# WHDY/SceneDepthEstimation

Hardware: AMD Instinct MI355X
Metric: Mpixel-disparities/sec (H*W*D cost voxels per second, end-to-end per pair) (higher is better)
Workload: dtype f32; 1 GPU; north_star; H=1024, W=1024, D=192, C=64, nlayers=5, pipeline=tower+cv_wta, global_batch=1, parallelism=pairdp1

## Files before the change

scenedepthestimation_amd/csrc/cv_row.hip:

```cpp
#include "cv_cert.h"

#include <algorithm>
#include <type_traits>

namespace sde {

constexpr int RW_S = 8;
constexpr float RW_SCALE = 256.0f;
constexpr float RW_K = 1.5e-5f;
constexpr float RW_ABS = 9.3132257e-10f;
constexpr float RW_NMAX = 127.0f;
typedef _Float16 rw_f16x8 __attribute__((ext_vector_type(8)));

__device__ __forceinline__ void rw_split(float x, _Float16 &h, _Float16 &l)
{
    const float xs = x * RW_SCALE;
    h = (_Float16)xs;
    l = (_Float16)(xs - (float)h);
}

constexpr int RW_T = 32;
constexpr int RW_WAVES = 8;
constexpr int RW_NX = RW_T * RW_WAVES;
constexpr int RW_NEW = RW_NX / RW_T;
// ... 244 lines not shown
#if CV_FASTSPLIT & 32
        const float xs[4] = {v[i].x * RW_SCALE, v[i].y * RW_SCALE, v[i].z * RW_SCALE, v[i].w * RW_SCALE};
        typedef _Float16 h2 __attribute__((ext_vector_type(2)));
        uint32_t hw[2], lw[2];
#pragma unroll
        for (int e = 0; e < 2; e++) {
            const h2 hh = {(_Float16)xs[2 * e], (_Float16)xs[2 * e + 1]};
            hw[e] = __builtin_bit_cast(uint32_t, hh);
            asm("v_fma_mixlo_f16 %0, %1, 1.0, -%2 op_sel_hi:[0,0,1]" : "=&v"(lw[e]) : "v"(xs[2 * e]), "v"(hw[e]));
            asm("v_fma_mixhi_f16 %0, %1, 1.0, -%2 op_sel:[0,0,1] op_sel_hi:[0,0,1]" : "+v"(lw[e]) : "v"(xs[2 * e + 1]), "v"(hw[e]));
        }
        *reinterpret_cast<uint2 *>(base) = uint2{hw[0], hw[1]};
        *reinterpret_cast<uint2 *>(base + 256 * 16) = uint2{lw[0], lw[1]};
#else
        _Float16 h0, h1, h2, h3, l0, l1, l2, l3;
        rw_split(v[i].x, h0, l0); rw_split(v[i].y, h1, l1); rw_split(v[i].z, h2, l2); rw_split(v[i].w, h3, l3);
        typedef _Float16 h4 __attribute__((ext_vector_type(4)));
        const h4 hv = {h0, h1, h2, h3}, lv = {l0, l1, l2, l3};
        *reinterpret_cast<uint2 *>(base) = __builtin_bit_cast(uint2, hv);
        *reinterpret_cast<uint2 *>(base + 256 * 16) = __builtin_bit_cast(uint2, lv);
#endif
        float ss = v[i].x * v[i].x + v[i].y * v[i].y + v[i].z * v[i].z + v[i].w * v[i].w;
        ss += rw_dpp<0xB1>(ss);
        ss += rw_dpp<0x4E>(ss);
        ss += rw_dpp<0x141>(ss);
        ss += rw_dpp<0x140>(ss);
        mx = max(mx, __float_as_uint(ss));
#if CV_FASTSPLIT & 16
        bad |= rw_nonfinite(ss);
#else
        bad |= rw_nonfinite(v[i].x) || rw_nonfinite(v[i].y) || rw_nonfinite(v[i].z) || rw_nonfinite(v[i].w);
#endif
    }
#pragma unroll
    for (int o = 1; o < 64; o <<= 1) mx = max(mx, (unsigned)__shfl_xor((int)mx, o, 64));
    const bool anybad = __ballot(bad) != 0;
    if (lane == 0) {
        tmax[slot] = mx;
        tbad[slot] = anybad ? 1u : 0u;
    }
}

template <bool WANT_MIN>
__global__ __launch_bounds__(512) void cv_wta_row2_kernel(const float *__restrict__ fl, const float *__restrict__ fr,
                                                          int H, int W, int d0, int d1, int tlo0, int nw, int nt,
                                                          float *__restrict__ out_min, int32_t *__restrict__ out_arg,
                                                          float *__restrict__ out_disp, unsigned *__restrict__ counter,
                                                          int32_t *__restrict__ list, const float *__restrict__ prev_min)
{
    extern __shared__ __attribute__((aligned(16))) uint4 rsm2[];
    uint4 *ring = rsm2;
    unsigned *tmax = reinterpret_cast<unsigned *>(ring + nt * 512);
    unsigned *tbad = tmax + nt;
    const int y = blockIdx.x;
    const int tid = threadIdx.x, lane = tid & 63;
    const int wave = __builtin_amdgcn_readfirstlane(tid >> 6);
    const int j = lane & 31, h = lane >> 5;
    const float *flrow = fl + (size_t)y * W * 64;
    const float *frrow = fr + (size_t)y * W * 64;
    const size_t rowpix = (size_t)y * W;
    const int nss = (W + R2_NX - 1) / R2_NX;
    auto slot_of = [&](int T) { int r = T % nt; return r < 0 ? r + nt : r; };

    if (wave >= 4) {
        const int sw = wave - 4;
        constexpr int PB = 4;
        float4 nv[8];
#pragma unroll
        for (int b = 0; b < 4 / PB; b++) {
            float4 pv[PB][8];
#pragma unroll
            for (int i = 0; i < PB; i++)
                if (sw + 4 * (PB * b + i) < nw) r2_load(frrow, W, tlo0 + sw + 4 * (PB * b + i), lane, pv[i]);
            if (b == 4 / PB - 1 && nss > 1) r2_load(frrow, W, tlo0 + nw + sw, lane, nv);
#pragma unroll
            for (int i = 0; i < PB; i++)
                if (sw + 4 * (PB * b + i) < nw) r2_store(ring, tmax, tbad, slot_of(tlo0 + sw + 4 * (PB * b + i)), lane, pv[i]);
        }
        __syncthreads();
        for (int k = 0; k < nss; k++) {
            if (k + 1 < nss) {
                const int T = tlo0 + R2_NEW * (k + 1) + nw - R2_NEW + sw;
                r2_store(ring, tmax, tbad, slot_of(T), lane, nv);
                if (k + 2 < nss) r2_load(frrow, W, T + R2_NEW, lane, nv);
            }
            __syncthreads();
        }
        return;
    }

    const int grp = wave & 3;
    float4 lraw[8];
    auto load_left = [&](int kk) {
        const int xx = kk * R2_NX + RW_T * grp + j;
        const float4 *src = reinterpret_cast<const float4 *>(flrow) + (size_t)(xx < W ? xx : 0) * 16 + 2 * h;
#pragma unroll
        for (int s2 = 0; s2 < 4; s2++) { lraw[2 * s2] = src[4 * s2]; lraw[2 * s2 + 1] = src[4 * s2 + 1]; }
    };
    load_left(0);
    __syncthreads();

    for (int k = 0; k < nss; k++) {
        const int tlo = tlo0 + R2_NEW * k;
        const bool more = k + 1 < nss;
        const int xb = k * R2_NX + RW_T * grp;
        const int x = xb + j;
        const bool xok = x < W;
        float best = -__builtin_inff(), second = -__builtin_inff();
        float wcost = -0.0f;
        int arg = -1;
        float nl = 0.0f;
        unsigned nmax2 = 0u, wbad = 0u;
        bool lbad = false;
        if (xb < W && xb + RW_T - 1 < d0) {
            if (more) load_left(k + 1);
        } else if (xb < W) {
            rw_f16x8 bh[4], bl[4];
            float ssl = 0.0f;
#if CV_FASTSPLIT & 1
            const float scl = RW_SCALE;
#pragma unroll
            for (int s2 = 0; s2 < 4; s2++) {
                const float4 a = lraw[2 * s2], b = lraw[2 * s2 + 1];
                const float v8[8] = {a.x, a.y, a.z, a.w, b.x, b.y, b.z, b.w};
                uint32_t hw[4], lw[4];
#pragma unroll
                for (int e = 0; e < 8; e += 2) {
                    const float x0 = v8[e] * scl, x1 = v8[e + 1] * scl;
                    typedef _Float16 h2 __attribute__((ext_vector_type(2)));
                    const h2 hh = {(_Float16)x0, (_Float16)x1};
                    const uint32_t hv = __builtin_bit_cast(uint32_t, hh);
                    uint32_t lv;
                    asm("v_fma_mixlo_f16 %0, %1, 1.0, -%2 op_sel_hi:[0,0,1]" : "=&v"(lv) : "v"(x0), "v"(hv));
                    asm("v_fma_mixhi_f16 %0, %1, 1.0, -%2 op_sel:[0,0,1] op_sel_hi:[0,0,1]" : "+v"(lv) : "v"(x1), "v"(hv));
                    hw[e / 2] = hv;
                    lw[e / 2] = lv;
                    ssl += v8[e] * v8[e];
                    ssl += v8[e + 1] * v8[e + 1];
                }
                bh[s2] = __builtin_bit_cast(rw_f16x8, uint4{hw[0], hw[1], hw[2], hw[3]});
                bl[s2] = __builtin_bit_cast(rw_f16x8, uint4{lw[0], lw[1], lw[2], lw[3]});
            }
#else
#pragma unroll
            for (int s2 = 0; s2 < 4; s2++) {
                const float4 a = lraw[2 * s2], b = lraw[2 * s2 + 1];
                const float v8[8] = {a.x, a.y, a.z, a.w, b.x, b.y, b.z, b.w};
#pragma unroll
                for (int e = 0; e < 8; e++) {
                    _Float16 hh, ll;
                    rw_split(v8[e], hh, ll);
                    bh[s2][e] = hh;
                    bl[s2][e] = ll;
                    ssl += v8[e] * v8[e];
                    if (!(CV_FASTSPLIT & 2)) lbad |= rw_nonfinite(v8[e]);
                }
            }
#endif
#if CV_FASTSPLIT & 2
#if CV_FASTSPLIT & 8
            ssl += __shfl_xor(ssl, 32, 64);
#else
            ssl += __builtin_bit_cast(float, __builtin_amdgcn_permlane32_swap(__float_as_uint(ssl), __float_as_uint(ssl),
                                                                              false, false)[1]);
#endif
            lbad = rw_nonfinite(ssl);
#else
            ssl += __shfl_xor(ssl, 32, 64);
            lbad |= __shfl_xor((int)lbad, 32, 64) != 0;
#endif
            nl = sqrtf(ssl) * FX_NORM_UP;
            if (more) load_left(k + 1);

            float b1[4], b2[4];
            int ag[4];
#pragma unroll
            for (int t = 0; t < 4; t++) { b1[t] = -__builtin_inff(); b2[t] = -__builtin_inff(); ag[t] = -1; }
            const int Ta = (xb - d1 + 1 + RW_T * 4096) / RW_T - 4096;
            const int Tb = (xb + 31 - d0 + RW_T * 4096) / RW_T - 4096;
            const int T0 = max(Ta, tlo), T1 = min(Tb, tlo + nw - 1);
            int slot = slot_of(T0);
            {
                const int n = T1 - T0 + 1;
                constexpr int PD = 1;
                rw_f16x8 fh[PD][4], fo[PD][4];
                fx_floatx16 A[2];
                auto nxt = [&](int sl2) { return sl2 + 1 == nt ? 0 : sl2 + 1; };
                auto frag = [&](int sl2, rw_f16x8 (&ah)[4], rw_f16x8 (&al)[4]) {
                    const uint4 *tp = ring + sl2 * 512;
#pragma unroll
                    for (int s2 = 0; s2 < 4; s2++) {
                        const int sl = fx_slot(j, 2 * s2 + h);
                        ah[s2] = __builtin_bit_cast(rw_f16x8, tp[sl]);
                        al[s2] = __builtin_bit_cast(rw_f16x8, tp[256 + sl]);
                    }
                };
                auto mfma = [&](int m, fx_floatx16 &acc, const rw_f16x8 (&ah)[4], const rw_f16x8 (&al)[4]) {
                    if (m == 0) acc = __builtin_amdgcn_mfma_f32_32x32x16_f16(al[0], bh[0], fx_floatx16{0}, 0, 0, 0);
                    else if (m < 8) acc = __builtin_amdgcn_mfma_f32_32x32x16_f16((m & 1) ? ah[m >> 1] : al[m >> 1],
                                                                                (m & 1) ? bl[m >> 1] : bh[m >> 1],
                                                                                acc, 0, 0, 0);
                    else acc = __builtin_amdgcn_mfma_f32_32x32x16_f16(ah[m - 8], bh[m - 8], acc, 0, 0, 0);
                };
                auto score1 = [&](const fx_floatx16 &acc, int r, auto mode_c, const int (&dk)[4]) {
                    constexpr int MODE = decltype(mode_c)::value;
                    const int tt = r & 3;
                    const bool in = MODE == 0   ? true
                                    : MODE == 1 ? dk[r >> 2] < d1 + tt
                                    : MODE == 3 ? dk[r >> 2] >= d0 + tt
                                                : (dk[r >> 2] - tt) >= d0 && (dk[r >> 2] - tt) < d1;
                    const float sc = in ? acc[r] : -__builtin_inff();
                    const bool gt = sc > b1[tt];
                    ag[tt] = gt ? dk[r >> 2] : ag[tt];
                    b2[tt] = __builtin_amdgcn_fmed3f(b1[tt], b2[tt], sc);
                    b1[tt] = fmaxf(b1[tt], sc);
                };
                auto step = [&](auto issue_c, auto load_c, int T, int sl2, const fx_floatx16 &acc, int nsl,
                                fx_floatx16 &accn, rw_f16x8 (&fbh)[4], rw_f16x8 (&fbl)[4], int lsl,
                                rw_f16x8 (&lbh)[4], rw_f16x8 (&lbl)[4]) {
                    constexpr bool issue = decltype(issue_c)::value, load = decltype(load_c)::value;
                    if (PD == 1 && issue) frag(nsl, fbh, fbl);
                    if (PD == 2 && load) frag(lsl, lbh, lbl);
                    nmax2 = max(nmax2, tmax[sl2]);
                    wbad |= tbad[sl2];
                    const int dt = xb - RW_T * T;
                    const bool lowok = dt - 31 >= d0, highok = dt + 31 < d1;
                    const int dl = dt + j - 4 * h;
                    int dk[4];
#pragma unroll
                    for (int k2 = 0; k2 < 4; k2++) dk[k2] = dl - 8 * k2;
                    constexpr int LD = CV_LEAD, RS = 16 - CV_LEAD;
                    auto body = [&](auto mode_c) {
#pragma unroll
                        for (int r = 0; r < LD; r++) score1(acc, r, mode_c, dk);
#pragma unroll
                        for (int m = 0; m < 12; m++) {
                            if (issue) mfma(m, accn, fbh, fbl);
#pragma unroll
                            for (int r = LD + (RS * m) / 12; r < LD + (RS * (m + 1)) / 12; r++)
                                score1(acc, r, mode_c, dk);
                        }
                    };
                    if (lowok && highok) {
                        asm volatile("");
                        body(std::integral_constant<int, 0>{});
                    } else if (!WANT_MIN && lowok) {
                        body(std::integral_constant<int, 1>{});
                    } else if (!WANT_MIN && highok) {
                        body(std::integral_constant<int, 3>{});
                    } else {
                        body(std::integral_constant<int, 2>{});
                    }
                };
                if (n > 0) {
                    using yes = std::integral_constant<bool, true>;
                    using no = std::integral_constant<bool, false>;
                    constexpr int B1 = PD - 1;
                    int sa = slot;
                    frag(sa, fh[0], fo[0]);
                    if (PD == 2 && n > 1) frag(nxt(sa), fh[B1], fo[B1]);
#pragma unroll
                    for (int m = 0; m < 12; m++) mfma(m, A[0], fh[0], fo[0]);
                    int i2 = 0;
                    for (; i2 + 3 < n; i2 += 2) {
                        const int sb = nxt(sa), sc2 = nxt(sb), sd = nxt(sc2);
                        step(yes{}, yes{}, T0 + i2, sa, A[0], sb, A[1], fh[B1], fo[B1], sc2, fh[0], fo[0]);
                        step(yes{}, yes{}, T0 + i2 + 1, sb, A[1], sc2, A[0], fh[0], fo[0], sd, fh[B1], fo[B1]);
                        sa = sc2;
                    }
                    const int sb = nxt(sa), sc2 = nxt(sb);
                    if (i2 + 2 < n) {
                        step(yes{}, yes{}, T0 + i2, sa, A[0], sb, A[1], fh[B1], fo[B1], sc2, fh[0], fo[0]);
                        step(yes{}, no{}, T0 + i2 + 1, sb, A[1], sc2, A[0], fh[0], fo[0], sc2, fh[B1], fo[B1]);
                        step(no{}, no{}, T0 + i2 + 2, sc2, A[0], sc2, A[1], fh[B1], fo[B1], sc2, fh[0], fo[0]);
                    } else if (i2 + 1 < n) {
                        step(yes{}, no{}, T0 + i2, sa, A[0], sb, A[1], fh[B1], fo[B1], sb, fh[0], fo[0]);
                        step(no{}, no{}, T0 + i2 + 1, sb, A[1], sb, A[0], fh[0], fo[0], sb, fh[B1], fo[B1]);
                    } else {
                        step(no{}, no{}, T0 + i2, sa, A[0], sa, A[1], fh[B1], fo[B1], sa, fh[0], fo[0]);
                    }
                }
            }
#pragma unroll
            for (int t = 0; t < 4; t++) ag[t] = ag[t] >= 0 ? ag[t] - t : -1;
            best = b1[0]; second = b2[0]; arg = ag[0];
#pragma unroll
            for (int t = 1; t < 4; t++) fx_merge(best, arg, second, b1[t], ag[t], b2[t]);
            {
#if CV_FASTSPLIT & 4
                auto up = [](uint32_t v) { return __builtin_amdgcn_permlane32_swap(v, v, false, false)[1]; };
                const float bb = __uint_as_float(up(__float_as_uint(best))), ss2 = __uint_as_float(up(__float_as_uint(second)));
                const int aa = (int)up((uint32_t)arg);
#else
                const float bb = __shfl_xor(best, 32, 64), ss2 = __shfl_xor(second, 32, 64);
                const int aa = __shfl_xor(arg, 32, 64);
#endif
                fx_merge(best, arg, second, bb, aa, ss2);
            }
            if constexpr (WANT_MIN) {
                const uint32_t lo_arg = __builtin_amdgcn_permlane32_swap((uint32_t)arg, (uint32_t)arg, false, false)[0];
                const int ab = h ? (int)lo_arg : arg;
                const int xr = x - ab;
                const bool ok = xok && ab >= 0 && xr >= 0;
                const float4 *la = reinterpret_cast<const float4 *>(flrow + (size_t)(xok ? x : 0) * 64) + h;
                const float4 *ra = reinterpret_cast<const float4 *>(frrow + (size_t)(ok ? xr : 0) * 64) + h;
                float4 lv[8], rv[8];
#pragma unroll
                for (int m = 0; m < 8; m++) {
                    lv[m] = la[2 * m];
                    rv[m] = ra[2 * m];
                }
                float a4[4];
#pragma unroll
                for (int m = 0; m < 8; m++) {
                    const float p4[4] = {lv[m].x * rv[m].x, lv[m].y * rv[m].y, lv[m].z * rv[m].z, lv[m].w * rv[m].w};
#pragma unroll
                    for (int e = 0; e < 4; e++) a4[e] = m == 0 ? p4[e] : a4[e] + p4[e];
                }
                const float half = (a4[0] + a4[1]) + (a4[2] + a4[3]);
                const float other = __uint_as_float(
                    __builtin_amdgcn_permlane32_swap(__float_as_uint(half), __float_as_uint(half), false, false)[1]);
                wcost = -(0.0f + (half + other));
            }
        }
        __syncthreads();
        if (xb < W && h == 0 && xok) {
            const float nr = sqrtf(__uint_as_float(nmax2)) * FX_NORM_UP;
            const float eps = (RW_K * nl * nr + RW_ABS * (nl + nr) + FX_ABS) * (RW_SCALE * RW_SCALE);
            const size_t p = rowpix + x;
            const bool none = x < d0;
            const bool fin = !lbad && !wbad && nl < RW_NMAX && nr < RW_NMAX;
            if (!none && fin && WANT_MIN && prev_min && best + 2.0f * eps < -prev_min[p] * (RW_SCALE * RW_SCALE)) {
                out_min[p] = __builtin_inff();
                if (out_arg) out_arg[p] = -1;
            } else if (none || (fin && (best - second) > 2.0f * eps && arg >= 0)) {
                if (none) arg = d0;
                if (WANT_MIN) {
                    float cost = -0.0f;
                    if (x - arg >= 0) cost = wcost;
                    out_min[p] = cost;
                }
                if (out_arg) out_arg[p] = arg;
                if (out_disp) out_disp[p] = (float)arg;
            } else {
                list[atomicAdd(counter, 1u)] = (int32_t)p;
            }
        }
    }
}

static void row_window(int d0, int d1, int &tlo0, int &ntw)
{
    auto fdiv = [](int a, int b) { return a >= 0 ? a / b : -((-a + b - 1) / b); };
    tlo0 = fdiv(-(d1 - 1), RW_T);
    const int thi0 = fdiv(RW_NX - 1 - d0, RW_T);
    ntw = thi0 - tlo0 + 1;
}

static size_t row_smem(int ntw) { return (size_t)ntw * 512 * 16 + (size_t)ntw * 8; }

static void row2_window(int d0, int d1, int &tlo0, int &nw)
{
    auto fdiv = [](int a, int b) { return a >= 0 ? a / b : -((-a + b - 1) / b); };
    tlo0 = fdiv(-(d1 - 1), RW_T);
    nw = fdiv(R2_NX - 1 - d0, RW_T) - tlo0 + 1;
}

static size_t row2_smem(int nt) { return row_smem(nt); }

static bool row2_supported(int d0, int d1)
{
    int tlo0 = 0, nw = 0;
    row2_window(d0, d1, tlo0, nw);
    return nw <= 14;
}

bool row_cert_supported(int d0, int d1)
{
    int tlo0 = 0, ntw = 0;
    row_window(d0, d1, tlo0, ntw);
    return ntw <= 18 || row2_supported(d0, d1);
}

void launch_row_cert(const float *fl, const float *fr, int H, int W, int d0, int d1, float *out_min, int32_t *out_arg,
                     float *out_disp, unsigned *counter, int32_t *list, hipStream_t st, const float *prev_min)
{
    static std::atomic<uint64_t> attr{0};
    constexpr int NT2 = 512;
    once_per_device(attr, [] {
        (void)hipFuncSetAttribute((const void *)cv_wta_row_kernel<true>, hipFuncAttributeMaxDynamicSharedMemorySize,
                                  150 * 1024);
        (void)hipFuncSetAttribute((const void *)cv_wta_row_kernel<false>, hipFuncAttributeMaxDynamicSharedMemorySize,
                                  150 * 1024);
        (void)hipFuncSetAttribute((const void *)cv_wta_row2_kernel<true>,
                                  hipFuncAttributeMaxDynamicSharedMemorySize, 150 * 1024);
        (void)hipFuncSetAttribute((const void *)cv_wta_row2_kernel<false>,
                                  hipFuncAttributeMaxDynamicSharedMemorySize, 150 * 1024);
    });
    if (row2_supported(d0, d1)) {
        int tlo0 = 0, nw = 0;
        row2_window(d0, d1, tlo0, nw);
        const int nt = nw + R2_NEW;
        if (out_min)
            cv_wta_row2_kernel<true><<<H, NT2, row2_smem(nt), st>>>(fl, fr, H, W, d0, d1, tlo0, nw, nt,
                                                                          out_min, out_arg, out_disp, counter, list,
                                                                          prev_min);
        else
            cv_wta_row2_kernel<false><<<H, NT2, row2_smem(nt), st>>>(fl, fr, H, W, d0, d1, tlo0, nw, nt,
                                                                           nullptr, out_arg, out_disp, counter, list,
                                                                           nullptr);
        return;
    }
    int tlo0 = 0, ntw = 0;
    row_window(d0, d1, tlo0, ntw);
    if (out_min)
        cv_wta_row_kernel<true><<<H, 512, row_smem(ntw), st>>>(fl, fr, H, W, d0, d1, tlo0, ntw, out_min, out_arg,
                                                               out_disp, counter, list);
    else
        cv_wta_row_kernel<false><<<H, 512, row_smem(ntw), st>>>(fl, fr, H, W, d0, d1, tlo0, ntw, nullptr, out_arg,
                                                                out_disp, counter, list);
}

}
```

scenedepthestimation_amd/csrc/sde_common.h:

```cpp
#pragma once

#include <hip/hip_runtime.h>
#include <stdint.h>

#include <atomic>
#include <type_traits>

#include "sde.h"

#define SDE_EXPORT extern "C" __attribute__((visibility("default")))

namespace sde {

static inline hipStream_t as_stream(void *s) { return reinterpret_cast<hipStream_t>(s); }

static inline int launch_status()
{
    hipError_t e = hipGetLastError();
    return e == hipSuccess ? SDE_OK : SDE_ERR_LAUNCH;
}

static inline int cdiv(int64_t a, int64_t b) { return (int)((a + b - 1) / b); }

template <typename F>
static inline bool once_per_device(std::atomic<uint64_t> &done, F fn)
{
    constexpr bool checked = std::is_same<decltype(fn()), bool>::value;
    int dev = 0;
    if (hipGetDevice(&dev) != hipSuccess || dev < 0 || dev >= 64) {
        if constexpr (checked) return fn();
        fn();
        return true;
    }
    const uint64_t bit = 1ull << dev;
    if (done.load(std::memory_order_acquire) & bit) return true;
    bool ok = true;
    if constexpr (checked) ok = fn();
    else fn();
    if (ok) done.fetch_or(bit, std::memory_order_acq_rel);
    return ok;
}

__device__ __forceinline__ int swz_row16(int row, int chunk) { return row * 16 + (chunk ^ (row & 15)); }

__device__ static float pw_prod_rec(const float *a, const float *b, int n)
{
    if (n < 8) {
        float res = 0.0f;
        for (int i = 0; i < n; i++) res += a[i] * b[i];
        return res;
    }
    if (n <= 128) {
        float r[8];
#pragma unroll
        for (int j = 0; j < 8; j++) r[j] = a[j] * b[j];
        int i = 8;
        for (; i < n - (n % 8); i += 8) {
#pragma unroll
            for (int j = 0; j < 8; j++) r[j] += a[i + j] * b[i + j];
        }
        float res = ((r[0] + r[1]) + (r[2] + r[3])) + ((r[4] + r[5]) + (r[6] + r[7]));
        for (; i < n; i++) res += a[i] * b[i];
        return res;
    }
    int n2 = n / 2;
    n2 -= n2 % 8;
    return pw_prod_rec(a, b, n2) + pw_prod_rec(a + n2, b + n2, n - n2);
}

__device__ __forceinline__ float np_neg_dot(const float *a, const float *b, int n)
{
    float s = 0.0f + pw_prod_rec(a, b, n);
    return -s;
}

__device__ __forceinline__ void argmin_merge(float &ma, int &aa, float mb, int ab)
{
    if (mb < ma || (mb == ma && ab < aa)) {
        ma = mb;
        aa = ab;
    }
}

}
```

scenedepthestimation_amd/csrc/tower.hip:

```cpp
#include "sde_common.h"

#include <atomic>

#include <vector>

#include <algorithm>
#include <cmath>
#include <cstring>
#include <type_traits>

namespace sde {

typedef float floatx16 __attribute__((ext_vector_type(16)));

constexpr int TW_TY = 8;
constexpr int TW_TX = 32;
constexpr int TW_IY = TW_TY + 2;
constexpr int TW_IX = TW_TX + 2;
constexpr int TW_NPIX = TW_IY * TW_IX;
constexpr int NF = 64;
constexpr int L1_FLOATS = NF + 9 * NF;
constexpr int LK_W = 9 * NF * NF;
constexpr int LK_F16 = NF + LK_W + 3 * LK_W / 2;
constexpr int LK_HDR = 8;
// ... 1289 lines not shown
    (void)hipFuncSetAttribute((const void *)conv64_mfma_kernel<false, false>, hipFuncAttributeMaxDynamicSharedMemorySize, TW_SMEM);
    (void)hipFuncSetAttribute((const void *)conv64_mfma_kernel<false, true>, hipFuncAttributeMaxDynamicSharedMemorySize, TW_SMEM);
#define SDE_X6P_ATTR1(F, L, I, O, H) (void)hipFuncSetAttribute((const void *)conv64_x6p_kernel<F, L, I, O, H>, \
                                                             hipFuncAttributeMaxDynamicSharedMemorySize, XP_SMEM)
#define SDE_X6P_ATTR(F, L, I, O) SDE_X6P_ATTR1(F, L, I, O, false); SDE_X6P_ATTR1(F, L, I, O, true)
    SDE_X6P_ATTR(true, false, false, true);
    SDE_X6P_ATTR(true, false, false, false);
    SDE_X6P_ATTR(true, true, false, false);
    SDE_X6P_ATTR(false, false, true, true);
    SDE_X6P_ATTR(false, false, false, false);
    SDE_X6P_ATTR(false, false, true, false);
    SDE_X6P_ATTR(false, false, false, true);
    SDE_X6P_ATTR(false, true, true, false);
    SDE_X6P_ATTR(false, true, false, false);
    (void)hipFuncSetAttribute((const void *)conv64_x6p_kernel<true, false, false, false, true, true>,
                              hipFuncAttributeMaxDynamicSharedMemorySize, XP_SMEM);
#undef SDE_X6P_ATTR1
#undef SDE_X6P_ATTR
#define SDE_H16_ATTR(L, I, O, S, ...) (void)hipFuncSetAttribute((const void *)conv64_h16_kernel<L, I, O, S, ##__VA_ARGS__>, \
                                                                hipFuncAttributeMaxDynamicSharedMemorySize, H16_SMEM)
    SDE_H16_ATTR(false, false, false, false, true, true);
    (void)hipFuncSetAttribute((const void *)conv64_h16q_kernel, hipFuncAttributeMaxDynamicSharedMemorySize, H16_SMEM);
    (void)hipFuncSetAttribute((const void *)conv64_h16_kernel<false, false, true, false, false, false, true>,
                              hipFuncAttributeMaxDynamicSharedMemorySize, H16_SMEM_FIRST);
    (void)hipFuncSetAttribute((const void *)conv64_h16_kernel<false, false, false, false, false, false, true>,
                              hipFuncAttributeMaxDynamicSharedMemorySize, H16_SMEM_FIRST);
    (void)hipFuncSetAttribute((const void *)conv64_h16_kernel<false, false, false, false, false, true, true>,
                              hipFuncAttributeMaxDynamicSharedMemorySize, H16_SMEM_FIRST);
    SDE_H16_ATTR(true, false, false, false, true, false);
    SDE_H16_ATTR(true, false, false, true, true, false);
    SDE_H16_ATTR(true, true, false, false);
    SDE_H16_ATTR(true, false, false, false);
    SDE_H16_ATTR(true, true, false, true);
    SDE_H16_ATTR(true, false, false, true);
    SDE_H16_ATTR(false, true, true, false);
    SDE_H16_ATTR(false, true, false, false);
    SDE_H16_ATTR(false, false, true, false);
    SDE_H16_ATTR(false, false, false, false);
#undef SDE_H16_ATTR
#define SDE_WINO_ATTR(L, I, O) (void)hipFuncSetAttribute((const void *)wino_kernel<L, I, O>, \
                                                         hipFuncAttributeMaxDynamicSharedMemorySize, WN_SMEM)
    SDE_WINO_ATTR(true, true, false);
    SDE_WINO_ATTR(true, false, false);
    SDE_WINO_ATTR(false, true, true);
    SDE_WINO_ATTR(false, true, false);
    SDE_WINO_ATTR(false, false, true);
    SDE_WINO_ATTR(false, false, false);
#undef SDE_WINO_ATTR
    });
}

static std::atomic<int> g_grid_cus{0};

static int cu_count()
{
    static int cached[64] = {0};
    int dev = 0;
    if (hipGetDevice(&dev) != hipSuccess || dev < 0 || dev >= 64) return 256;
    if (!cached[dev]) {
        int n = 0;
        if (hipDeviceGetAttribute(&n, hipDeviceAttributeMultiprocessorCount, dev) != hipSuccess || n <= 0) n = 256;
        cached[dev] = n;
    }
    const int g = g_grid_cus.load(std::memory_order_relaxed);
    return g > 0 ? std::min(g, cached[dev]) : cached[dev];
}

static void launch_layer(const float *in, int Hin, int Win, const float *packed, int nlayers, int layer, float *out,
                         int flags, uint16_t *ohi, uint16_t *olo, float *onrm, bool in_cb, bool out_cb,
                         const float *in_amax, float *out_amax, hipStream_t st, int nimg = 1, int64_t in_stride = 0,
                         int64_t out_stride = 0, int amax_stride = 0, bool in_sp = false, bool out_sp = false)
{
    set_tower_attrs();
    const bool last = (layer == nlayers);
    const bool f16 = (flags & SDE_TOWER_F16X3) != 0;
    const bool x6 = f16 || (flags & SDE_TOWER_BF16X6) != 0;
    const float *w1 = packed;
    const float *wk = packed + L1_FLOATS + (int64_t)(layer - 2) * LK_FLOATS;
    const int hout = Hin - (layer == 2 ? 4 : 2), wout = Win - (layer == 2 ? 4 : 2);
    const bool wino_fits = (int64_t)Hin * Win * 256 < ((int64_t)1 << 32) &&
                           (int64_t)hout * wout * 256 < ((int64_t)1 << 32);
    if (f16 && layer >= 3 && !ohi && !onrm && (flags & SDE_TOWER_WINOGRAD) && wino_fits) {
        XpBatch bt;
        bt.tiles_x = cdiv(wout, WN_TX);
        bt.tiles_img = bt.tiles_x * cdiv(hout, WN_TY);
        bt.ntiles = bt.tiles_img * nimg;
        bt.in_stride = in_stride;
        bt.out_stride = out_stride;
        bt.pix_stride = (int64_t)hout * wout;
        bt.amax_stride = amax_stride;
        const int grid = std::min(bt.ntiles, cu_count());
#define SDE_WINO(L, I, O) wino_kernel<L, I, O><<<grid, 512, WN_SMEM, st>>>(in, Hin, Win, wk, out, hout, wout, bt, \
                                                                          in_amax, out_amax)
        if (last) { if (in_cb) SDE_WINO(true, true, false); else SDE_WINO(true, false, false); }
        else if (in_cb) { if (out_cb) SDE_WINO(false, true, true); else SDE_WINO(false, true, false); }
        else { if (out_cb) SDE_WINO(false, false, true); else SDE_WINO(false, false, false); }
#undef SDE_WINO
        return;
    }
    if (f16 && layer == 2 && !last && !(flags & SDE_TOWER_MFMA32) && SDE_H16_L2) {
        XpBatch bt;
        bt.tiles_x = cdiv(wout, XP_TX);
        bt.tiles_img = bt.tiles_x * cdiv(hout, XP_TY);
        bt.ntiles = bt.tiles_img * nimg;
        bt.in_stride = in_stride;
        bt.out_stride = out_stride;
        bt.pix_stride = (int64_t)hout * wout;
// ... 304 lines not shown
```

Measured before the change: 120,300 Mpixel-disparities/s.

## Make row cost-volume kernel persistent and prefetch next row across iterations

Launches the row-based cost-volume WTA kernel with one block per CU instead of one per image row, with each block looping over rows in a grid-stride fashion. The producer waves prefetch the next row's right-feature tiles during the last column step, and in the non-min variant the consumer waves prefetch the next row's left features. This targets block launch and ramp-up cost and hides the initial load latency of each row. It also makes cu_count a shared non-static function. Possible downsides are load imbalance when H is not a multiple of the grid and higher register pressure from the extra prefetch buffers.

```diff
diff --git a/scenedepthestimation_amd/csrc/cv_row.hip b/scenedepthestimation_amd/csrc/cv_row.hip
--- a/scenedepthestimation_amd/csrc/cv_row.hip
+++ b/scenedepthestimation_amd/csrc/cv_row.hip
@@ -320,298 +320,317 @@
     uint4 *ring = rsm2;
     unsigned *tmax = reinterpret_cast<unsigned *>(ring + nt * 512);
     unsigned *tbad = tmax + nt;
-    const int y = blockIdx.x;
+    const int ystep = gridDim.x;
     const int tid = threadIdx.x, lane = tid & 63;
     const int wave = __builtin_amdgcn_readfirstlane(tid >> 6);
-    const int j = lane & 31, h = lane >> 5;
-    const float *flrow = fl + (size_t)y * W * 64;
-    const float *frrow = fr + (size_t)y * W * 64;
-    const size_t rowpix = (size_t)y * W;
     const int nss = (W + R2_NX - 1) / R2_NX;
     auto slot_of = [&](int T) { int r = T % nt; return r < 0 ? r + nt : r; };
 
     if (wave >= 4) {
         const int sw = wave - 4;
         constexpr int PB = 4;
-        float4 nv[8];
-#pragma unroll
-        for (int b = 0; b < 4 / PB; b++) {
-            float4 pv[PB][8];
+        float4 pv[PB][8], nv[8];
+        auto load_row = [&](const float *row) {
+            int ln = lane;
+            asm volatile("" : "+v"(ln));
 #pragma unroll
             for (int i = 0; i < PB; i++)
-                if (sw + 4 * (PB * b + i) < nw) r2_load(frrow, W, tlo0 + sw + 4 * (PB * b + i), lane, pv[i]);
-            if (b == 4 / PB - 1 && nss > 1) r2_load(frrow, W, tlo0 + nw + sw, lane, nv);
+                if (sw + 4 * i < nw) r2_load(row, W, tlo0 + sw + 4 * i, ln, pv[i]);
+            if (nss > 1) r2_load(row, W, tlo0 + nw + sw, ln, nv);
+        };
+        load_row(fr + (size_t)blockIdx.x * W * 64);
+        for (int y = blockIdx.x; y < H; y += ystep) {
+            const float *frrow = fr + (size_t)y * W * 64;
+            const bool nextrow = y + ystep < H;
 #pragma unroll
             for (int i = 0; i < PB; i++)
-                if (sw + 4 * (PB * b + i) < nw) r2_store(ring, tmax, tbad, slot_of(tlo0 + sw + 4 * (PB * b + i)), lane, pv[i]);
-        }
-        __syncthreads();
-        for (int k = 0; k < nss; k++) {
-            if (k + 1 < nss) {
-                const int T = tlo0 + R2_NEW * (k + 1) + nw - R2_NEW + sw;
-                r2_store(ring, tmax, tbad, slot_of(T), lane, nv);
-                if (k + 2 < nss) r2_load(frrow, W, T + R2_NEW, lane, nv);
+                if (sw + 4 * i < nw) r2_store(ring, tmax, tbad, slot_of(tlo0 + sw + 4 * i), lane, pv[i]);
+            __syncthreads();
+            for (int k = 0; k < nss; k++) {
+                if (k + 1 < nss) {
+                    const int T = tlo0 + R2_NEW * (k + 1) + nw - R2_NEW + sw;
+                    r2_store(ring, tmax, tbad, slot_of(T), lane, nv);
+                    if (k + 2 < nss) r2_load(frrow, W, T + R2_NEW, lane, nv);
+                }
+                if (nextrow && k == (nss > 1 ? nss - 2 : 0)) load_row(fr + (size_t)(y + ystep) * W * 64);
+                __syncthreads();
             }
-            __syncthreads();
         }
         return;
     }
 
     const int grp = wave & 3;
+    int ln = lane;
     float4 lraw[8];
-    auto load_left = [&](int kk) {
-        const int xx = kk * R2_NX + RW_T * grp + j;
-        const float4 *src = reinterpret_cast<const float4 *>(flrow) + (size_t)(xx < W ? xx : 0) * 16 + 2 * h;
+    auto load_left = [&](const float *row, int kk) {
+        const int xx = kk * R2_NX + RW_T * grp + (ln & 31);
+        const float4 *src = reinterpret_cast<const float4 *>(row) + (size_t)(xx < W ? xx : 0) * 16 + 2 * (ln >> 5);
 #pragma unroll
         for (int s2 = 0; s2 < 4; s2++) { lraw[2 * s2] = src[4 * s2]; lraw[2 * s2 + 1] = src[4 * s2 + 1]; }
     };
-    load_left(0);
-    __syncthreads();
-
-    for (int k = 0; k < nss; k++) {
-        const int tlo = tlo0 + R2_NEW * k;
-        const bool more = k + 1 < nss;
-        const int xb = k * R2_NX + RW_T * grp;
-        const int x = xb + j;
-        const bool xok = x < W;
-        float best = -__builtin_inff(), second = -__builtin_inff();
-        float wcost = -0.0f;
-        int arg = -1;
-        float nl = 0.0f;
-        unsigned nmax2 = 0u, wbad = 0u;
-        bool lbad = false;
-        if (xb < W && xb + RW_T - 1 < d0) {
-            if (more) load_left(k + 1);
-        } else if (xb < W) {
-            rw_f16x8 bh[4], bl[4];
-            float ssl = 0.0f;
+    constexpr bool LEFT_AHEAD = !WANT_MIN;
+    if (LEFT_AHEAD) load_left(fl + (size_t)blockIdx.x * W * 64, 0);
+    for (int y = blockIdx.x; y < H; y += ystep) {
+        const float *flrow = fl + (size_t)y * W * 64;
+        const float *frrow = fr + (size_t)y * W * 64;
+        const size_t rowpix = (size_t)y * W;
+        const bool nextrow = y + ystep < H;
+        asm volatile("" : "+v"(ln));
+        const int j = ln & 31, h = ln >> 5;
+        if (!LEFT_AHEAD) load_left(flrow, 0);
+        __syncthreads();
+
+        for (int k = 0; k < nss; k++) {
+            const int tlo = tlo0 + R2_NEW * k;
+            const bool more = k + 1 < nss;
+            const int xb = k * R2_NX + RW_T * grp;
+            const int x = xb + j;
+            const bool xok = x < W;
+            float best = -__builtin_inff(), second = -__builtin_inff();
+            float wcost = -0.0f;
+            int arg = -1;
+            float nl = 0.0f;
+            unsigned nmax2 = 0u, wbad = 0u;
+            bool lbad = false;
+            auto next_left = [&]() {
+                if (more) load_left(flrow, k + 1);
+                else if (LEFT_AHEAD && nextrow) load_left(fl + (size_t)(y + ystep) * W * 64, 0);
+            };
+            if (xb >= W) {
+                next_left();
+            } else if (xb + RW_T - 1 < d0) {
+                next_left();
+            } else {
+                rw_f16x8 bh[4], bl[4];
+                float ssl = 0.0f;
 #if CV_FASTSPLIT & 1
-            const float scl = RW_SCALE;
-#pragma unroll
-            for (int s2 = 0; s2 < 4; s2++) {
-                const float4 a = lraw[2 * s2], b = lraw[2 * s2 + 1];
-                const float v8[8] = {a.x, a.y, a.z, a.w, b.x, b.y, b.z, b.w};
-                uint32_t hw[4], lw[4];
-#pragma unroll
-                for (int e = 0; e < 8; e += 2) {
-                    const float x0 = v8[e] * scl, x1 = v8[e + 1] * scl;
-                    typedef _Float16 h2 __attribute__((ext_vector_type(2)));
-                    const h2 hh = {(_Float16)x0, (_Float16)x1};
-                    const uint32_t hv = __builtin_bit_cast(uint32_t, hh);
-                    uint32_t lv;
-                    asm("v_fma_mixlo_f16 %0, %1, 1.0, -%2 op_sel_hi:[0,0,1]" : "=&v"(lv) : "v"(x0), "v"(hv));
-                    asm("v_fma_mixhi_f16 %0, %1, 1.0, -%2 op_sel:[0,0,1] op_sel_hi:[0,0,1]" : "+v"(lv) : "v"(x1), "v"(hv));
-                    hw[e / 2] = hv;
-                    lw[e / 2] = lv;
-                    ssl += v8[e] * v8[e];
-                    ssl += v8[e + 1] * v8[e + 1];
-                }
-                bh[s2] = __builtin_bit_cast(rw_f16x8, uint4{hw[0], hw[1], hw[2], hw[3]});
-                bl[s2] = __builtin_bit_cast(rw_f16x8, uint4{lw[0], lw[1], lw[2], lw[3]});
-            }
+                const float scl = RW_SCALE;
+#pragma unroll
+                for (int s2 = 0; s2 < 4; s2++) {
+                    const float4 a = lraw[2 * s2], b = lraw[2 * s2 + 1];
+                    const float v8[8] = {a.x, a.y, a.z, a.w, b.x, b.y, b.z, b.w};
+                    uint32_t hw[4], lw[4];
+#pragma unroll
+                    for (int e = 0; e < 8; e += 2) {
+                        const float x0 = v8[e] * scl, x1 = v8[e + 1] * scl;
+                        typedef _Float16 h2 __attribute__((ext_vector_type(2)));
+                        const h2 hh = {(_Float16)x0, (_Float16)x1};
+                        const uint32_t hv = __builtin_bit_cast(uint32_t, hh);
+                        uint32_t lv;
+                        asm("v_fma_mixlo_f16 %0, %1, 1.0, -%2 op_sel_hi:[0,0,1]" : "=&v"(lv) : "v"(x0), "v"(hv));
+                        asm("v_fma_mixhi_f16 %0, %1, 1.0, -%2 op_sel:[0,0,1] op_sel_hi:[0,0,1]" : "+v"(lv) : "v"(x1), "v"(hv));
+                        hw[e / 2] = hv;
+                        lw[e / 2] = lv;
+                        ssl += v8[e] * v8[e];
+                        ssl += v8[e + 1] * v8[e + 1];
+                    }
+                    bh[s2] = __builtin_bit_cast(rw_f16x8, uint4{hw[0], hw[1], hw[2], hw[3]});
+                    bl[s2] = __builtin_bit_cast(rw_f16x8, uint4{lw[0], lw[1], lw[2], lw[3]});
+                }
 #else
 #pragma unroll
-            for (int s2 = 0; s2 < 4; s2++) {
-                const float4 a = lraw[2 * s2], b = lraw[2 * s2 + 1];
-                const float v8[8] = {a.x, a.y, a.z, a.w, b.x, b.y, b.z, b.w};
-#pragma unroll
-                for (int e = 0; e < 8; e++) {
-                    _Float16 hh, ll;
-                    rw_split(v8[e], hh, ll);
-                    bh[s2][e] = hh;
-                    bl[s2][e] = ll;
-                    ssl += v8[e] * v8[e];
-                    if (!(CV_FASTSPLIT & 2)) lbad |= rw_nonfinite(v8[e]);
-                }
-            }
+                for (int s2 = 0; s2 < 4; s2++) {
+                    const float4 a = lraw[2 * s2], b = lraw[2 * s2 + 1];
+                    const float v8[8] = {a.x, a.y, a.z, a.w, b.x, b.y, b.z, b.w};
+#pragma unroll
+                    for (int e = 0; e < 8; e++) {
+                        _Float16 hh, ll;
+                        rw_split(v8[e], hh, ll);
+                        bh[s2][e] = hh;
+                        bl[s2][e] = ll;
+                        ssl += v8[e] * v8[e];
+                        if (!(CV_FASTSPLIT & 2)) lbad |= rw_nonfinite(v8[e]);
+                    }
+                }
 #endif
 #if CV_FASTSPLIT & 2
 #if CV_FASTSPLIT & 8
-            ssl += __shfl_xor(ssl, 32, 64);
+                ssl += __shfl_xor(ssl, 32, 64);
 #else
-            ssl += __builtin_bit_cast(float, __builtin_amdgcn_permlane32_swap(__float_as_uint(ssl), __float_as_uint(ssl),
-                                                                              false, false)[1]);
+                ssl += __builtin_bit_cast(float, __builtin_amdgcn_permlane32_swap(__float_as_uint(ssl), __float_as_uint(ssl),
+                                                                                  false, false)[1]);
 #endif
-            lbad = rw_nonfinite(ssl);
+                lbad = rw_nonfinite(ssl);
 #else
-            ssl += __shfl_xor(ssl, 32, 64);
-            lbad |= __shfl_xor((int)lbad, 32, 64) != 0;
+                ssl += __shfl_xor(ssl, 32, 64);
+                lbad |= __shfl_xor((int)lbad, 32, 64) != 0;
 #endif
-            nl = sqrtf(ssl) * FX_NORM_UP;
-            if (more) load_left(k + 1);
-
-            float b1[4], b2[4];
-            int ag[4];
-#pragma unroll
-            for (int t = 0; t < 4; t++) { b1[t] = -__builtin_inff(); b2[t] = -__builtin_inff(); ag[t] = -1; }
-            const int Ta = (xb - d1 + 1 + RW_T * 4096) / RW_T - 4096;
-            const int Tb = (xb + 31 - d0 + RW_T * 4096) / RW_T - 4096;
-            const int T0 = max(Ta, tlo), T1 = min(Tb, tlo + nw - 1);
-            int slot = slot_of(T0);
-            {
-                const int n = T1 - T0 + 1;
-                constexpr int PD = 1;
-                rw_f16x8 fh[PD][4], fo[PD][4];
-                fx_floatx16 A[2];
-                auto nxt = [&](int sl2) { return sl2 + 1 == nt ? 0 : sl2 + 1; };
-                auto frag = [&](int sl2, rw_f16x8 (&ah)[4], rw_f16x8 (&al)[4]) {
-                    const uint4 *tp = ring + sl2 * 512;
-#pragma unroll
-                    for (int s2 = 0; s2 < 4; s2++) {
-                        const int sl = fx_slot(j, 2 * s2 + h);
-                        ah[s2] = __builtin_bit_cast(rw_f16x8, tp[sl]);
-                        al[s2] = __builtin_bit_cast(rw_f16x8, tp[256 + sl]);
-                    }
-                };
-                auto mfma = [&](int m, fx_floatx16 &acc, const rw_f16x8 (&ah)[4], const rw_f16x8 (&al)[4]) {
-                    if (m == 0) acc = __builtin_amdgcn_mfma_f32_32x32x16_f16(al[0], bh[0], fx_floatx16{0}, 0, 0, 0);
-                    else if (m < 8) acc = __builtin_amdgcn_mfma_f32_32x32x16_f16((m & 1) ? ah[m >> 1] : al[m >> 1],
-                                                                                (m & 1) ? bl[m >> 1] : bh[m >> 1],
-                                                                                acc, 0, 0, 0);
-                    else acc = __builtin_amdgcn_mfma_f32_32x32x16_f16(ah[m - 8], bh[m - 8], acc, 0, 0, 0);
-                };
-                auto score1 = [&](const fx_floatx16 &acc, int r, auto mode_c, const int (&dk)[4]) {
-                    constexpr int MODE = decltype(mode_c)::value;
-                    const int tt = r & 3;
-                    const bool in = MODE == 0   ? true
-                                    : MODE == 1 ? dk[r >> 2] < d1 + tt
-                                    : MODE == 3 ? dk[r >> 2] >= d0 + tt
-                                                : (dk[r >> 2] - tt) >= d0 && (dk[r >> 2] - tt) < d1;
-                    const float sc = in ? acc[r] : -__builtin_inff();
-                    const bool gt = sc > b1[tt];
-                    ag[tt] = gt ? dk[r >> 2] : ag[tt];
-                    b2[tt] = __builtin_amdgcn_fmed3f(b1[tt], b2[tt], sc);
-                    b1[tt] = fmaxf(b1[tt], sc);
-                };
-                auto step = [&](auto issue_c, auto load_c, int T, int sl2, const fx_floatx16 &acc, int nsl,
-                                fx_floatx16 &accn, rw_f16x8 (&fbh)[4], rw_f16x8 (&fbl)[4], int lsl,
-                                rw_f16x8 (&lbh)[4], rw_f16x8 (&lbl)[4]) {
-                    constexpr bool issue = decltype(issue_c)::value, load = decltype(load_c)::value;
-                    if (PD == 1 && issue) frag(nsl, fbh, fbl);
-                    if (PD == 2 && load) frag(lsl, lbh, lbl);
-                    nmax2 = max(nmax2, tmax[sl2]);
-                    wbad |= tbad[sl2];
-                    const int dt = xb - RW_T * T;
-                    const bool lowok = dt - 31 >= d0, highok = dt + 31 < d1;
-                    const int dl = dt + j - 4 * h;
-                    int dk[4];
-#pragma unroll
-                    for (int k2 = 0; k2 < 4; k2++) dk[k2] = dl - 8 * k2;
-                    constexpr int LD = CV_LEAD, RS = 16 - CV_LEAD;
-                    auto body = [&](auto mode_c) {
-#pragma unroll
-                        for (int r = 0; r < LD; r++) score1(acc, r, mode_c, dk);
-#pragma unroll
-                        for (int m = 0; m < 12; m++) {
-                            if (issue) mfma(m, accn, fbh, fbl);
-#pragma unroll
-                            for (int r = LD + (RS * m) / 12; r < LD + (RS * (m + 1)) / 12; r++)
-                                score1(acc, r, mode_c, dk);
+                nl = sqrtf(ssl) * FX_NORM_UP;
+                next_left();
+
+                float b1[4], b2[4];
+                int ag[4];
+#pragma unroll
+                for (int t = 0; t < 4; t++) { b1[t] = -__builtin_inff(); b2[t] = -__builtin_inff(); ag[t] = -1; }
+                const int Ta = (xb - d1 + 1 + RW_T * 4096) / RW_T - 4096;
+                const int Tb = (xb + 31 - d0 + RW_T * 4096) / RW_T - 4096;
+                const int T0 = max(Ta, tlo), T1 = min(Tb, tlo + nw - 1);
+                int slot = slot_of(T0);
+                {
+                    const int n = T1 - T0 + 1;
+                    constexpr int PD = 1;
+                    rw_f16x8 fh[PD][4], fo[PD][4];
+                    fx_floatx16 A[2];
+                    auto nxt = [&](int sl2) { return sl2 + 1 == nt ? 0 : sl2 + 1; };
+                    auto frag = [&](int sl2, rw_f16x8 (&ah)[4], rw_f16x8 (&al)[4]) {
+                        const uint4 *tp = ring + sl2 * 512;
+#pragma unroll
+                        for (int s2 = 0; s2 < 4; s2++) {
+                            const int sl = fx_slot(j, 2 * s2 + h);
+                            ah[s2] = __builtin_bit_cast(rw_f16x8, tp[sl]);
+                            al[s2] = __builtin_bit_cast(rw_f16x8, tp[256 + sl]);
                         }
                     };
-                    if (lowok && highok) {
-                        asm volatile("");
-                        body(std::integral_constant<int, 0>{});
-                    } else if (!WANT_MIN && lowok) {
-                        body(std::integral_constant<int, 1>{});
-                    } else if (!WANT_MIN && highok) {
-                        body(std::integral_constant<int, 3>{});
-                    } else {
-                        body(std::integral_constant<int, 2>{});
+                    auto mfma = [&](int m, fx_floatx16 &acc, const rw_f16x8 (&ah)[4], const rw_f16x8 (&al)[4]) {
+                        if (m == 0) acc = __builtin_amdgcn_mfma_f32_32x32x16_f16(al[0], bh[0], fx_floatx16{0}, 0, 0, 0);
+                        else if (m < 8) acc = __builtin_amdgcn_mfma_f32_32x32x16_f16((m & 1) ? ah[m >> 1] : al[m >> 1],
+                                                                                    (m & 1) ? bl[m >> 1] : bh[m >> 1],
+                                                                                    acc, 0, 0, 0);
+                        else acc = __builtin_amdgcn_mfma_f32_32x32x16_f16(ah[m - 8], bh[m - 8], acc, 0, 0, 0);
+                    };
+                    auto score1 = [&](const fx_floatx16 &acc, int r, auto mode_c, const int (&dk)[4]) {
+                        constexpr int MODE = decltype(mode_c)::value;
+                        const int tt = r & 3;
+                        const bool in = MODE == 0   ? true
+                                        : MODE == 1 ? dk[r >> 2] < d1 + tt
+                                        : MODE == 3 ? dk[r >> 2] >= d0 + tt
+                                                    : (dk[r >> 2] - tt) >= d0 && (dk[r >> 2] - tt) < d1;
+                        const float sc = in ? acc[r] : -__builtin_inff();
+                        const bool gt = sc > b1[tt];
+                        ag[tt] = gt ? dk[r >> 2] : ag[tt];
+                        b2[tt] = __builtin_amdgcn_fmed3f(b1[tt], b2[tt], sc);
+                        b1[tt] = fmaxf(b1[tt], sc);
+                    };
+                    auto step = [&](auto issue_c, auto load_c, int T, int sl2, const fx_floatx16 &acc, int nsl,
+                                    fx_floatx16 &accn, rw_f16x8 (&fbh)[4], rw_f16x8 (&fbl)[4], int lsl,
+                                    rw_f16x8 (&lbh)[4], rw_f16x8 (&lbl)[4]) {
+                        constexpr bool issue = decltype(issue_c)::value, load = decltype(load_c)::value;
+                        if (PD == 1 && issue) frag(nsl, fbh, fbl);
+                        if (PD == 2 && load) frag(lsl, lbh, lbl);
+                        nmax2 = max(nmax2, tmax[sl2]);
+                        wbad |= tbad[sl2];
+                        const int dt = xb - RW_T * T;
+                        const bool lowok = dt - 31 >= d0, highok = dt + 31 < d1;
+                        const int dl = dt + j - 4 * h;
+                        int dk[4];
+#pragma unroll
+                        for (int k2 = 0; k2 < 4; k2++) dk[k2] = dl - 8 * k2;
+                        constexpr int LD = CV_LEAD, RS = 16 - CV_LEAD;
+                        auto body = [&](auto mode_c) {
+#pragma unroll
+                            for (int r = 0; r < LD; r++) score1(acc, r, mode_c, dk);
+#pragma unroll
+                            for (int m = 0; m < 12; m++) {
+                                if (issue) mfma(m, accn, fbh, fbl);
+#pragma unroll
+                                for (int r = LD + (RS * m) / 12; r < LD + (RS * (m + 1)) / 12; r++)
+                                    score1(acc, r, mode_c, dk);
+                            }
+                        };
+                        if (lowok && highok) {
+                            asm volatile("");
+                            body(std::integral_constant<int, 0>{});
+                        } else if (!WANT_MIN && lowok) {
+                            body(std::integral_constant<int, 1>{});
+                        } else if (!WANT_MIN && highok) {
+                            body(std::integral_constant<int, 3>{});
+                        } else {
+                            body(std::integral_constant<int, 2>{});
+                        }
+                    };
+                    if (n > 0) {
+                        using yes = std::integral_constant<bool, true>;
+                        using no = std::integral_constant<bool, false>;
+                        constexpr int B1 = PD - 1;
+                        int sa = slot;
+                        frag(sa, fh[0], fo[0]);
+                        if (PD == 2 && n > 1) frag(nxt(sa), fh[B1], fo[B1]);
+#pragma unroll
+                        for (int m = 0; m < 12; m++) mfma(m, A[0], fh[0], fo[0]);
+                        int i2 = 0;
+                        for (; i2 + 3 < n; i2 += 2) {
+                            const int sb = nxt(sa), sc2 = nxt(sb), sd = nxt(sc2);
+                            step(yes{}, yes{}, T0 + i2, sa, A[0], sb, A[1], fh[B1], fo[B1], sc2, fh[0], fo[0]);
+                            step(yes{}, yes{}, T0 + i2 + 1, sb, A[1], sc2, A[0], fh[0], fo[0], sd, fh[B1], fo[B1]);
+                            sa = sc2;
+                        }
+                        const int sb = nxt(sa), sc2 = nxt(sb);
+                        if (i2 + 2 < n) {
+                            step(yes{}, yes{}, T0 + i2, sa, A[0], sb, A[1], fh[B1], fo[B1], sc2, fh[0], fo[0]);
+                            step(yes{}, no{}, T0 + i2 + 1, sb, A[1], sc2, A[0], fh[0], fo[0], sc2, fh[B1], fo[B1]);
+                            step(no{}, no{}, T0 + i2 + 2, sc2, A[0], sc2, A[1], fh[B1], fo[B1], sc2, fh[0], fo[0]);
+                        } else if (i2 + 1 < n) {
+                            step(yes{}, no{}, T0 + i2, sa, A[0], sb, A[1], fh[B1], fo[B1], sb, fh[0], fo[0]);
+                            step(no{}, no{}, T0 + i2 + 1, sb, A[1], sb, A[0], fh[0], fo[0], sb, fh[B1], fo[B1]);
+                        } else {
+                            step(no{}, no{}, T0 + i2, sa, A[0], sa, A[1], fh[B1], fo[B1], sa, fh[0], fo[0]);
+                        }
                     }
-                };
-                if (n > 0) {
-                    using yes = std::integral_constant<bool, true>;
-                    using no = std::integral_constant<bool, false>;
-                    constexpr int B1 = PD - 1;
-                    int sa = slot;
-                    frag(sa, fh[0], fo[0]);
-                    if (PD == 2 && n > 1) frag(nxt(sa), fh[B1], fo[B1]);
-#pragma unroll
-                    for (int m = 0; m < 12; m++) mfma(m, A[0], fh[0], fo[0]);
-                    int i2 = 0;
-                    for (; i2 + 3 < n; i2 += 2) {
-                        const int sb = nxt(sa), sc2 = nxt(sb), sd = nxt(sc2);
-                        step(yes{}, yes{}, T0 + i2, sa, A[0], sb, A[1], fh[B1], fo[B1], sc2, fh[0], fo[0]);
-                        step(yes{}, yes{}, T0 + i2 + 1, sb, A[1], sc2, A[0], fh[0], fo[0], sd, fh[B1], fo[B1]);
-                        sa = sc2;
+                }
+#pragma unroll
+                for (int t = 0; t < 4; t++) ag[t] = ag[t] >= 0 ? ag[t] - t : -1;
+                best = b1[0]; second = b2[0]; arg = ag[0];
+#pragma unroll
+                for (int t = 1; t < 4; t++) fx_merge(best, arg, second, b1[t], ag[t], b2[t]);
+                {
+#if CV_FASTSPLIT & 4
+                    auto up = [](uint32_t v) { return __builtin_amdgcn_permlane32_swap(v, v, false, false)[1]; };
+                    const float bb = __uint_as_float(up(__float_as_uint(best))), ss2 = __uint_as_float(up(__float_as_uint(second)));
+                    const int aa = (int)up((uint32_t)arg);
+#else
+                    const float bb = __shfl_xor(best, 32, 64), ss2 = __shfl_xor(second, 32, 64);
+                    const int aa = __shfl_xor(arg, 32, 64);
+#endif
+                    fx_merge(best, arg, second, bb, aa, ss2);
+                }
+                if constexpr (WANT_MIN) {
+                    const uint32_t lo_arg = __builtin_amdgcn_permlane32_swap((uint32_t)arg, (uint32_t)arg, false, false)[0];
+                    const int ab = h ? (int)lo_arg : arg;
+                    const int xr = x - ab;
+                    const bool ok = xok && ab >= 0 && xr >= 0;
+                    const float4 *la = reinterpret_cast<const float4 *>(flrow + (size_t)(xok ? x : 0) * 64) + h;
+                    const float4 *ra = reinterpret_cast<const float4 *>(frrow + (size_t)(ok ? xr : 0) * 64) + h;
+                    float4 lv[8], rv[8];
+#pragma unroll
+                    for (int m = 0; m < 8; m++) {
+                        lv[m] = la[2 * m];
+                        rv[m] = ra[2 * m];
                     }
-                    const int sb = nxt(sa), sc2 = nxt(sb);
-                    if (i2 + 2 < n) {
-                        step(yes{}, yes{}, T0 + i2, sa, A[0], sb, A[1], fh[B1], fo[B1], sc2, fh[0], fo[0]);
-                        step(yes{}, no{}, T0 + i2 + 1, sb, A[1], sc2, A[0], fh[0], fo[0], sc2, fh[B1], fo[B1]);
-                        step(no{}, no{}, T0 + i2 + 2, sc2, A[0], sc2, A[1], fh[B1], fo[B1], sc2, fh[0], fo[0]);
-                    } else if (i2 + 1 < n) {
-                        step(yes{}, no{}, T0 + i2, sa, A[0], sb, A[1], fh[B1], fo[B1], sb, fh[0], fo[0]);
-                        step(no{}, no{}, T0 + i2 + 1, sb, A[1], sb, A[0], fh[0], fo[0], sb, fh[B1], fo[B1]);
-                    } else {
-                        step(no{}, no{}, T0 + i2, sa, A[0], sa, A[1], fh[B1], fo[B1], sa, fh[0], fo[0]);
+                    float a4[4];
+#pragma unroll
+                    for (int m = 0; m < 8; m++) {
+                        const float p4[4] = {lv[m].x * rv[m].x, lv[m].y * rv[m].y, lv[m].z * rv[m].z, lv[m].w * rv[m].w};
+#pragma unroll
+                        for (int e = 0; e < 4; e++) a4[e] = m == 0 ? p4[e] : a4[e] + p4[e];
                     }
+                    const float half = (a4[0] + a4[1]) + (a4[2] + a4[3]);
+                    const float other = __uint_as_float(
+                        __builtin_amdgcn_permlane32_swap(__float_as_uint(half), __float_as_uint(half), false, false)[1]);
+                    wcost = -(0.0f + (half + other));
                 }
             }
-#pragma unroll
-            for (int t = 0; t < 4; t++) ag[t] = ag[t] >= 0 ? ag[t] - t : -1;
-            best = b1[0]; second = b2[0]; arg = ag[0];
-#pragma unroll
-            for (int t = 1; t < 4; t++) fx_merge(best, arg, second, b1[t], ag[t], b2[t]);
-            {
-#if CV_FASTSPLIT & 4
-                auto up = [](uint32_t v) { return __builtin_amdgcn_permlane32_swap(v, v, false, false)[1]; };
-                const float bb = __uint_as_float(up(__float_as_uint(best))), ss2 = __uint_as_float(up(__float_as_uint(second)));
-                const int aa = (int)up((uint32_t)arg);
-#else
-                const float bb = __shfl_xor(best, 32, 64), ss2 = __shfl_xor(second, 32, 64);
-                const int aa = __shfl_xor(arg, 32, 64);
-#endif
-                fx_merge(best, arg, second, bb, aa, ss2);
-            }
-            if constexpr (WANT_MIN) {
-                const uint32_t lo_arg = __builtin_amdgcn_permlane32_swap((uint32_t)arg, (uint32_t)arg, false, false)[0];
-                const int ab = h ? (int)lo_arg : arg;
-                const int xr = x - ab;
-                const bool ok = xok && ab >= 0 && xr >= 0;
-                const float4 *la = reinterpret_cast<const float4 *>(flrow + (size_t)(xok ? x : 0) * 64) + h;
-                const float4 *ra = reinterpret_cast<const float4 *>(frrow + (size_t)(ok ? xr : 0) * 64) + h;
-                float4 lv[8], rv[8];
-#pragma unroll
-                for (int m = 0; m < 8; m++) {
-                    lv[m] = la[2 * m];
-                    rv[m] = ra[2 * m];
-                }
-                float a4[4];
-#pragma unroll
-                for (int m = 0; m < 8; m++) {
-                    const float p4[4] = {lv[m].x * rv[m].x, lv[m].y * rv[m].y, lv[m].z * rv[m].z, lv[m].w * rv[m].w};
-#pragma unroll
-                    for (int e = 0; e < 4; e++) a4[e] = m == 0 ? p4[e] : a4[e] + p4[e];
-                }
-                const float half = (a4[0] + a4[1]) + (a4[2] + a4[3]);
-                const float other = __uint_as_float(
-                    __builtin_amdgcn_permlane32_swap(__float_as_uint(half), __float_as_uint(half), false, false)[1]);
-                wcost = -(0.0f + (half + other));
-            }
-        }
-        __syncthreads();
-        if (xb < W && h == 0 && xok) {
-            const float nr = sqrtf(__uint_as_float(nmax2)) * FX_NORM_UP;
-            const float eps = (RW_K * nl * nr + RW_ABS * (nl + nr) + FX_ABS) * (RW_SCALE * RW_SCALE);
-            const size_t p = rowpix + x;
-            const bool none = x < d0;
-            const bool fin = !lbad && !wbad && nl < RW_NMAX && nr < RW_NMAX;
-            if (!none && fin && WANT_MIN && prev_min && best + 2.0f * eps < -prev_min[p] * (RW_SCALE * RW_SCALE)) {
-                out_min[p] = __builtin_inff();
-                if (out_arg) out_arg[p] = -1;
-            } else if (none || (fin && (best - second) > 2.0f * eps && arg >= 0)) {
-                if (none) arg = d0;
-                if (WANT_MIN) {
-                    float cost = -0.0f;
-                    if (x - arg >= 0) cost = wcost;
-                    out_min[p] = cost;
-                }
-                if (out_arg) out_arg[p] = arg;
-                if (out_disp) out_disp[p] = (float)arg;
-            } else {
-                list[atomicAdd(counter, 1u)] = (int32_t)p;
+            __syncthreads();
+            if (xb < W && h == 0 && xok) {
+                const float nr = sqrtf(__uint_as_float(nmax2)) * FX_NORM_UP;
+                const float eps = (RW_K * nl * nr + RW_ABS * (nl + nr) + FX_ABS) * (RW_SCALE * RW_SCALE);
+                const size_t p = rowpix + x;
+                const bool none = x < d0;
+                const bool fin = !lbad && !wbad && nl < RW_NMAX && nr < RW_NMAX;
+                if (!none && fin && WANT_MIN && prev_min && best + 2.0f * eps < -prev_min[p] * (RW_SCALE * RW_SCALE)) {
+                    out_min[p] = __builtin_inff();
+                    if (out_arg) out_arg[p] = -1;
+                } else if (none || (fin && (best - second) > 2.0f * eps && arg >= 0)) {
+                    if (none) arg = d0;
+                    if (WANT_MIN) {
+                        float cost = -0.0f;
+                        if (x - arg >= 0) cost = wcost;
+                        out_min[p] = cost;
+                    }
+                    if (out_arg) out_arg[p] = arg;
+                    if (out_disp) out_disp[p] = (float)arg;
+                } else {
+                    list[atomicAdd(counter, 1u)] = (int32_t)p;
+                }
             }
         }
     }
@@ -669,14 +688,15 @@
         int tlo0 = 0, nw = 0;
         row2_window(d0, d1, tlo0, nw);
         const int nt = nw + R2_NEW;
+        const int grid = std::min(H, cu_count());
         if (out_min)
-            cv_wta_row2_kernel<true><<<H, NT2, row2_smem(nt), st>>>(fl, fr, H, W, d0, d1, tlo0, nw, nt,
-                                                                          out_min, out_arg, out_disp, counter, list,
-                                                                          prev_min);
+            cv_wta_row2_kernel<true><<<grid, NT2, row2_smem(nt), st>>>(fl, fr, H, W, d0, d1, tlo0, nw, nt,
+                                                                             out_min, out_arg, out_disp, counter, list,
+                                                                             prev_min);
         else
-            cv_wta_row2_kernel<false><<<H, NT2, row2_smem(nt), st>>>(fl, fr, H, W, d0, d1, tlo0, nw, nt,
-                                                                           nullptr, out_arg, out_disp, counter, list,
-                                                                           nullptr);
+            cv_wta_row2_kernel<false><<<grid, NT2, row2_smem(nt), st>>>(fl, fr, H, W, d0, d1, tlo0, nw, nt,
+                                                                              nullptr, out_arg, out_disp, counter, list,
+                                                                              nullptr);
         return;
     }
     int tlo0 = 0, ntw = 0;
diff --git a/scenedepthestimation_amd/csrc/sde_common.h b/scenedepthestimation_amd/csrc/sde_common.h
--- a/scenedepthestimation_amd/csrc/sde_common.h
+++ b/scenedepthestimation_amd/csrc/sde_common.h
@@ -41,6 +41,8 @@
     return ok;
 }
 
+int cu_count();
+
 __device__ __forceinline__ int swz_row16(int row, int chunk) { return row * 16 + (chunk ^ (row & 15)); }
 
 __device__ static float pw_prod_rec(const float *a, const float *b, int n)
diff --git a/scenedepthestimation_amd/csrc/tower.hip b/scenedepthestimation_amd/csrc/tower.hip
--- a/scenedepthestimation_amd/csrc/tower.hip
+++ b/scenedepthestimation_amd/csrc/tower.hip
@@ -1365,7 +1365,7 @@
 
 static std::atomic<int> g_grid_cus{0};
 
-static int cu_count()
+int sde::cu_count()
 {
     static int cached[64] = {0};
     int dev = 0;
```

Measured after the change: 121,000 Mpixel-disparities/s, median of 6. Within noise of the previous version (+0.6%).
